# symek/facedeform

Hardware: AMD Instinct MI355X
Metric: deformed Mverts/sec at 256 ctrl pts, 1/2/4/8 MI355X vs host-CPU ref (higher is better)
Workload: dtype f32

## Files before the change

facedeform_amd/csrc/fd_capi.hip:

```cpp
#include <atomic>
#include <cstdarg>
#include <cstdio>
#include <cstdlib>
#include <cstring>
#include <initializer_list>
#include <new>

#include "fd_internal.h"

using namespace fd;

struct GraphKey {
    int M, kind, term, nparams;
    double params[4];
    const void *A, *rest, *rec32;
};

struct fd_batch;
struct fd_ctx {
    int device = 0;
    hipStream_t own_stream = nullptr;
    hipStream_t stream_ = nullptr;
    int eval_precision = FD_EVAL_FP32;
    int eval_variant = 0;
    int output = FD_OUTPUT_POSITION;
    int solver = FD_SOLVER_AUTO;
    int imported_layers = 0;
    uint64_t rig_build_id = 0;
    const float *rest_src = nullptr;
    bool prefer_lu = false;
    unsigned long long model_gen = 0;
    bool last_spd = false;
    bool last_nopivot = false;
    bool last_reg = false;

    int M = 0, kind = FD_KERNEL_GAUSSIAN_QNN, term = FD_TERM_LINEAR, nparams = 0;
    double params[4] = {1.0, 5.0, 0.0, 0.0};
    bool points_set = false;
    bool build_pending = false;
    bool built = false;
    bool have_report = false;
    fd_report report{};
    bool have_factor = false;
    bool factor_grouped = false;
    bool deltas_only = false;
    hipGraphExec_t resolve_exec = nullptr;

    int cap_M = 0;
    int cap_npad = 0;
    int cap_records = 0;
    float *d_rest = nullptr, *d_delta = nullptr;
    double *d_centres = nullptr, *d_radii = nullptr, *d_W = nullptr;
    double *d_A = nullptr, *d_X = nullptr;
    int *d_ipiv = nullptr, *d_moves = nullptr;
    Rec32 *d_rec32 = nullptr;
    Rec64 *d_rec64 = nullptr;
    MfmaTile *d_tiles = nullptr;
    MfmaTileH *d_tiles16 = nullptr;
    double *d_ns = nullptr;
    DevModel *d_model = nullptr;
    DevModel *h_model = nullptr;
    BatchSlot *d_slot = nullptr;
    BatchSlot h_slot{};
    uint64_t alloc_gen = 0;
    hipEvent_t wait_event = nullptr;
    hipStream_t wait_stream = nullptr;
    struct fd_batch *wait_batch = nullptr;
    hipEvent_t tev0 = nullptr, tev_mid = nullptr, tev1 = nullptr;
    ModelHeader *h_header = nullptr;
    int *h_status = nullptr;
    int *d_status_alias = nullptr;
    hipEvent_t status_ev = nullptr;
    hipEvent_t status_poll = nullptr;
    bool status_inflight = false;
    int sticky_rc = FD_OK;

    int64_t cap_N = 0;
    float *d_P = nullptr, *d_dist2 = nullptr, *d_fall = nullptr;
    float *d_tu = nullptr, *d_tv = nullptr, *d_nrm = nullptr;
    int64_t cap_vec = 0, cap_vecP = 0;
    float *d_vec = nullptr, *d_vecP = nullptr;
    int64_t mesh_N = 0, mesh_cap = 0;
    bool mesh_has_dist2 = false, mesh_has_frames = false;
    float *m_P = nullptr, *m_dist2 = nullptr, *m_tu = nullptr, *m_tv = nullptr, *m_nrm = nullptr;
    float *m_out = nullptr, *m_fall = nullptr;

    hipEvent_t ev0 = nullptr, ev_mid = nullptr, ev1 = nullptr;

    hipGraphExec_t build_exec = nullptr;
    bool use_graph = true;
    GraphKey graph_key{}, resolve_key{};
    char err[512] = {0};
};

struct ShotScratch {
    void *d = nullptr;
    size_t cap = 0;
    hipEvent_t consumed_ev = nullptr;
    bool consumed = false;
    hipEvent_t eval_ev = nullptr;
    bool eval_pending = false;
};

struct fd_batch {
    int n = 0;
    int device = 0;
    fd_ctx *ctxs[kMaxBatch] = {};
    uint64_t gens[kMaxBatch] = {};
    BatchSlot *d_slots = nullptr;
    PointSrc src{};
    bool have_src = false;
    hipEvent_t ev0 = nullptr, ev_mid = nullptr, ev1 = nullptr;
    hipGraphExec_t exec = nullptr;
    bool use_graph = true;
    GraphKey key{};
    hipStream_t waited_stream = nullptr;
    hipEvent_t status_ev = nullptr;
    struct SharedSet {
        void *d_wtiles = nullptr, *d_frames = nullptr;
        size_t cap_wtiles = 0, cap_frames = 0;
        hipEvent_t packed_ev = nullptr;
        hipEvent_t eval_ev = nullptr;
        hipEvent_t eval_done = nullptr;
        bool eval_pending = false;
    } sets[2];
    int *h_mismatch = nullptr;
    int eval_cus = 0;
    int shared_factor = 0;
    double *d_fac = nullptr;
    int last_shared_factor = 0;
    void *d_mlfac = nullptr;
    size_t cap_mlfac = 0;
    int cur_set = 0;
    bool packed_valid = false;
    bool prepared = false;
    unsigned long long prep_gen[kMaxBatch] = {0};
    float *prep_P_out[kMaxBatch] = {nullptr};
    float *prep_fall[kMaxBatch] = {nullptr};
    bool prep_has_fall = false;
    hipEvent_t fallback_ev = nullptr;
    ShotScratch s64;
    ShotScratch sml;
    ShotScratch sml64;
    hipEvent_t group_ev = nullptr;
    bool lean = false;
    hipEvent_t consumed_override = nullptr;
    char err[512] = {0};
};


static thread_local char g_err[512] = {0};

static void set_err(fd_ctx *ctx, const char *fmt, ...)
{
    char *dst = ctx ? ctx->err : g_err;
    va_list ap;
    va_start(ap, fmt);
    vsnprintf(dst, 512, fmt, ap);
    va_end(ap);
}

static hipStream_t cur_stream(fd_ctx *ctx)
{
    if (ctx->stream_) return ctx->stream_;
    if (!ctx->own_stream && hipStreamCreateWithFlags(&ctx->own_stream, hipStreamNonBlocking) != hipSuccess) {
        (void)hipGetLastError();
        ctx->own_stream = nullptr;
    }
    return ctx->own_stream;
}

#define FD_HIP(ctx, call)                                                               \
    do {                                                                                \
        hipError_t e_ = (call);                                                         \
        if (e_ != hipSuccess) {                                                         \
            set_err(ctx, "%s failed: %s (%s:%d)", #call, hipGetErrorString(e_), __FILE__, __LINE__); \
            return FD_E_DEVICE;                                                         \
        }                                                                               \
    } while (0)

static int use_device(fd_ctx *ctx)
{
    int cur = -1;
    FD_HIP(ctx, hipGetDevice(&cur));
    if (cur != ctx->device) FD_HIP(ctx, hipSetDevice(ctx->device));
    return FD_OK;
}

template <typename T>
static int dev_alloc(fd_ctx *ctx, T **p, size_t count)
{
    if (*p) { (void)hipFree(*p); *p = nullptr; }
    if (count == 0) count = 1;
    hipError_t e = hipMalloc((void **)p, count * sizeof(T));
    if (e != hipSuccess) {
        *p = nullptr;
        set_err(ctx, "hipMalloc(%zu bytes) failed: %s", count * sizeof(T), hipGetErrorString(e));
        return FD_E_NOMEM;
    }
    return FD_OK;
}

static int order_of(const fd_ctx *ctx) { return ctx->M + term_cols(ctx->term); }
static int ml_layers(const fd_ctx *ctx) { return ctx->kind == FD_KERNEL_GAUSSIAN_ML ? (int)ctx->params[1] : 0; }
static int model_centres(const fd_ctx *ctx) { return ctx->kind == FD_KERNEL_GAUSSIAN_ML ? ctx->M * ml_layers(ctx) : ctx->M; }
static int eval_kind(const fd_ctx *ctx) { return ctx->kind == FD_KERNEL_GAUSSIAN_ML ? FD_KERNEL_GAUSSIAN_QNN : ctx->kind; }
static int record_layers(const fd_ctx *ctx) { return ctx->kind == FD_KERNEL_GAUSSIAN_ML ? ml_layers(ctx) : ctx->imported_layers; }

static int ensure_records_capacity(fd_ctx *ctx, int n)
{
    int rc;
    if (n > ctx->cap_records) {
        const int npad = round_up(n, kRecPad);
        if ((rc = dev_alloc(ctx, &ctx->d_centres, (size_t)n * 3))) return rc;
        if ((rc = dev_alloc(ctx, &ctx->d_radii, (size_t)n))) return rc;
        if ((rc = dev_alloc(ctx, &ctx->d_W, (size_t)(n + 4) * 3))) return rc;
        if ((rc = dev_alloc(ctx, &ctx->d_rec32, (size_t)npad))) return rc;
        if ((rc = dev_alloc(ctx, &ctx->d_rec64, (size_t)npad))) return rc;
        if ((rc = dev_alloc(ctx, &ctx->d_tiles, (size_t)npad / 16))) return rc;
        if ((rc = dev_alloc(ctx, &ctx->d_tiles16, (size_t)npad / 16))) return rc;
        ctx->cap_records = n;
    }
    return FD_OK;
}

static int ensure_model_capacity(fd_ctx *ctx, int M)
{
// ... 1183 lines not shown
    if (!on_device) FD_HIP(ctx, hipStreamSynchronize(cur_stream(ctx)));
    ctx->have_factor = false;
    ctx->deltas_only = false;
    ++ctx->model_gen;
    ctx->points_set = false;
    ctx->rig_build_id = 0;
    ctx->rest_src = h.rig_token ? (const float *)(uintptr_t)(h.rig_token | 1u) : nullptr;
    ctx->build_pending = false;
    ctx->built = true;
    fd_report r{};
    r.terminationtype = 1;
    r.n = order_of(ctx);
    ctx->report = r;
    ctx->have_report = true;
    return FD_OK;
}

static void batch_err(fd_batch *b, const char *fmt, ...)
{
    char *dst = b ? b->err : g_err;
    va_list ap;
    va_start(ap, fmt);
    vsnprintf(dst, 512, fmt, ap);
    va_end(ap);
}

fd_batch *fd_batch_create(fd_ctx *const *ctxs, int n)
{
    if (!ctxs || n <= 0 || n > kMaxBatch) { set_err(nullptr, "fd_batch_create: need 1..%d contexts", kMaxBatch); return nullptr; }
    for (int i = 0; i < n; ++i) {
        if (!ctxs[i] || ctxs[i]->device != ctxs[0]->device) { set_err(nullptr, "fd_batch_create: contexts must exist and share one device"); return nullptr; }
        for (int j = 0; j < i; ++j)
            if (ctxs[j] == ctxs[i]) { set_err(nullptr, "fd_batch_create: context listed twice"); return nullptr; }
    }
    fd_batch *b = new (std::nothrow) fd_batch();
    if (!b) { set_err(nullptr, "fd_batch_create: out of host memory"); return nullptr; }
    b->n = n;
    b->device = ctxs[0]->device;
    for (int i = 0; i < n; ++i) b->ctxs[i] = ctxs[i];
    bool ok = hipSetDevice(b->device) == hipSuccess;
    ok = ok && hipMalloc((void **)&b->d_slots, sizeof(BatchSlot) * (size_t)n) == hipSuccess;
    ok = ok && hipEventCreate(&b->ev0) == hipSuccess && hipEventCreate(&b->ev_mid) == hipSuccess &&
         hipEventCreate(&b->ev1) == hipSuccess;
    ok = ok && hipEventCreateWithFlags(&b->status_ev, hipEventDisableTiming) == hipSuccess;
    ok = ok && hipHostMalloc((void **)&b->h_mismatch, sizeof(int), hipHostMallocMapped) == hipSuccess;
    if (ok) *b->h_mismatch = 0;
    if (!ok) {
        set_err(nullptr, "fd_batch_create: device resource allocation failed: %s", hipGetErrorString(hipGetLastError()));
        fd_batch_destroy(b);
        return nullptr;
    }
    return b;
}

static void shot_free(ShotScratch &sc)
{
    if (sc.d) (void)hipFree(sc.d);
    if (sc.consumed_ev) (void)hipEventDestroy(sc.consumed_ev);
    if (sc.eval_ev) (void)hipEventDestroy(sc.eval_ev);
}

void fd_batch_destroy(fd_batch *b)
{
    if (!b) return;
    (void)hipSetDevice(b->device);
    for (int i = 0; i < b->n; ++i) {
        fd_ctx *c = b->ctxs[i];
        if (c && c->wait_event == b->ev1) {
            if (c->wait_stream) (void)hipStreamSynchronize(c->wait_stream);
            c->wait_event = nullptr; c->wait_stream = nullptr; c->wait_batch = nullptr;
        }
        if (c && c->tev0 == b->ev0) { c->tev0 = c->ev0; c->tev_mid = c->ev_mid; c->tev1 = c->ev1; }
        if (c && (c->status_poll == b->status_ev || c->status_poll == b->ev1)) { c->status_poll = c->status_ev; c->status_inflight = false; }
    }
    if (b->status_ev) (void)hipEventDestroy(b->status_ev);
    if (b->exec) (void)hipGraphExecDestroy(b->exec);
    if (b->d_slots) (void)hipFree(b->d_slots);
    for (auto &st : b->sets) {
        if (st.d_wtiles) (void)hipFree(st.d_wtiles);
        if (st.d_frames) (void)hipFree(st.d_frames);
        if (st.packed_ev) (void)hipEventDestroy(st.packed_ev);
        if (st.eval_ev) (void)hipEventDestroy(st.eval_ev);
    }
    if (b->d_fac) (void)hipFree(b->d_fac);
    if (b->d_mlfac) (void)hipFree(b->d_mlfac);
    if (b->fallback_ev) (void)hipEventDestroy(b->fallback_ev);
    for (ShotScratch *sc : {&b->s64, &b->sml, &b->sml64}) shot_free(*sc);
    if (b->group_ev) (void)hipEventDestroy(b->group_ev);
    if (b->h_mismatch) (void)hipHostFree(b->h_mismatch);
    if (b->ev0) (void)hipEventDestroy(b->ev0);
    if (b->ev_mid) (void)hipEventDestroy(b->ev_mid);
    if (b->ev1) (void)hipEventDestroy(b->ev1);
    delete b;
}

const char *fd_batch_last_error(const fd_batch *b) { return b ? b->err : g_err; }

int fd_batch_set_points_dev(fd_batch *b, const float *const *d_rest_xyz, const float *const *d_delta_xyz, int M)
{
    if (!b || !d_rest_xyz || !d_delta_xyz) return FD_E_INVALID;
    if (M <= 0 || M + 4 > kMaxOrder) { batch_err(b, "fd_batch_set_points_dev: M = %d outside 1..%d", M, kMaxOrder - 4); return FD_E_INVALID; }
    b->prepared = false;
    if (b->h_mismatch && *b->h_mismatch != 0) {
        const int who = *b->h_mismatch - 1;
        *b->h_mismatch = 0;
        batch_err(b, "shared-rig evaluation of the previous group: context %d was built on other rest points than context 0 (same "
                     "address, other contents); its frame was passed through", who);
        return FD_E_INVALID;
    }
    for (int i = 0; i < b->n; ++i)
        if (!d_rest_xyz[i] || !d_delta_xyz[i]) { batch_err(b, "fd_batch_set_points_dev: null array for context %d", i); return FD_E_INVALID; }
    for (int i = 0; i < b->n; ++i) {
        fd_ctx *c = b->ctxs[i];
        int rc = use_device(c);
        if (!rc) rc = ensure_model_capacity(c, M);
        if (rc) { batch_err(b, "context %d: %s", i, c->err); return rc; }
        c->M = M;
        c->points_set = true;
        c->built = false;
        c->build_pending = false;
        c->have_factor = false;
        c->deltas_only = false;
        c->rest_src = d_rest_xyz[i];
        c->rig_build_id = 0;
        b->src.rest[i] = d_rest_xyz[i];
        b->src.delta[i] = d_delta_xyz[i];
    }
    b->have_src = true;
    return FD_OK;
}

int fd_batch_build_async(fd_batch *b, void *hip_stream)
{
    if (!b) return FD_E_INVALID;
    b->prepared = false;
    fd_ctx *c0 = b->ctxs[0];
    int rc = use_device(c0);
    if (rc) { batch_err(b, "%s", c0->err); return rc; }
    hipStream_t stream = hip_stream ? (hipStream_t)hip_stream : cur_stream(c0);
    for (int i = 0; i < b->n; ++i) {
        fd_ctx *c = b->ctxs[i];
        if (!c->points_set) { batch_err(b, "fd_batch_build: context %d has no control points", i); return FD_E_INVALID; }
        c->imported_layers = 0;
        if (!same_model(c, c0)) {
            batch_err(b, "fd_batch_build: context %d differs from context 0 in M, kernel, parameters or term", i);
            return FD_E_INVALID;
        }
    }
    const int npad = round_up(order_of(c0), 32);
    bool table_stale = false;
    for (int i = 0; i < b->n; ++i) {
        fd_ctx *c = b->ctxs[i];
        const bool grew = npad > c->cap_npad;
        if ((rc = ensure_solver_capacity(c, npad)) || (rc = ensure_records_capacity(c, model_centres(c))) || (rc = sync_slot(c))) {
            batch_err(b, "context %d: %s", i, c->err);
            return rc;
        }
        if (grew) {
            const size_t cols = (size_t)c->cap_npad + kRhsCols + 16;
            hipError_t e = hipMemsetAsync(c->d_A, 0, sizeof(double) * (size_t)c->cap_npad * cols, stream);
            if (e != hipSuccess) { batch_err(b, "hipMemsetAsync failed: %s", hipGetErrorString(e)); return FD_E_DEVICE; }
        }
        if (b->gens[i] != c->alloc_gen) table_stale = true;
    }
    if (table_stale) {
        BatchSlot tab[kMaxBatch];
// ... 9 lines not shown
    bb.reg_front = (b->eval_cus <= 0 || b->eval_cus >= (int)device_cus()) ? 1 : 0;
    bb.group_panels = b->n >= 4 ? 1 : 0;

    bool same_rest_launch = b->have_src;
    for (int i = 1; i < b->n && same_rest_launch; ++i) same_rest_launch = b->src.rest[i] == b->src.rest[0];
    bool shared_ml = b->shared_factor != 0 && bb.ml_layers > 0 && same_rest_launch && ml_shared_applies(bb.M, bb.ml_layers, b->n);
    if (shared_ml && ml_shared_init() != hipSuccess) { (void)hipGetLastError(); shared_ml = false; }
    if (shared_ml && ml_shared_scratch_bytes(bb) > b->cap_mlfac) {
        if (b->d_mlfac) (void)hipFree(b->d_mlfac);
        b->d_mlfac = nullptr; b->cap_mlfac = 0;
        if (hipMalloc(&b->d_mlfac, ml_shared_scratch_bytes(bb)) != hipSuccess) { (void)hipGetLastError(); b->d_mlfac = nullptr; shared_ml = false; }
        else b->cap_mlfac = ml_shared_scratch_bytes(bb);
    }

    const GraphKey key = graph_key(c0, (bb.spd << 9) | (bb.small << 10) | (bb.reg << 11) | (bb.nopivot << 12), false);
    if (!bb.reg && !shared_ml && b->use_graph &&
        ensure_graph(stream, &b->exec, &b->key, key, [&] { return launch_build(bb, stream, nullptr); }) != hipSuccess)
        b->use_graph = false;
#define FD_BHIP(call)                                                                         \
    do {                                                                                      \
        hipError_t e_ = (call);                                                               \
        if (e_ != hipSuccess) { batch_err(b, "%s failed: %s", #call, hipGetErrorString(e_)); return FD_E_DEVICE; } \
    } while (0)
    const bool shared_fac_ok = same_rest_launch;
    bool shared_fac = b->shared_factor != 0 && bb.reg && shared_fac_ok && b->n > 1;
    if (shared_fac && !b->d_fac && hipMalloc((void **)&b->d_fac, sizeof(double) * reg_factor_doubles()) != hipSuccess) {
        (void)hipGetLastError(); b->d_fac = nullptr; shared_fac = false;
    }
    b->last_shared_factor = (shared_fac || shared_ml) ? 1 : 0;
    if (!b->lean) FD_BHIP(hipEventRecord(b->ev0, stream));
    if (shared_fac) {
        FD_BHIP(launch_build_reg_shared(bb, stream, &b->src, nullptr, b->d_fac));
        b->have_src = false;
    } else if (bb.reg) {
        FD_BHIP(launch_build_reg(bb, stream, b->have_src ? &b->src : nullptr, nullptr));
        b->have_src = false;
    } else {
    FD_BHIP(launch_prepare(bb, stream, b->have_src ? &b->src : nullptr));
    b->have_src = false;
    if (shared_ml) {
        FD_BHIP(hipEventRecord(b->ev_mid, stream));
        FD_BHIP(launch_build_ml_shared(bb, stream, b->d_mlfac));
    } else if (b->use_graph && b->exec) {
        FD_BHIP(hipEventRecord(b->ev_mid, stream));
        FD_BHIP(hipGraphLaunch(b->exec, stream));
    } else {
        FD_BHIP(launch_build(bb, stream, b->ev_mid));
    }
    }
    if (!b->lean) FD_BHIP(hipEventRecord(b->ev1, stream));
    b->waited_stream = nullptr;
#undef FD_BHIP
    static std::atomic<uint64_t> build_ids{0};
    const uint64_t this_build = same_rest_launch ? ++build_ids : 0;
    hipEvent_t t0 = b->lean ? nullptr : b->ev0, t_mid = b->lean ? nullptr : (bb.reg ? b->ev0 : b->ev_mid), t1 = b->lean ? nullptr : b->ev1;
    for (int i = 0; i < b->n; ++i) note_build_enqueued(b->ctxs[i], b->ev1, stream, b, t0, t_mid, t1, &bb, this_build);
    arm_status(b->ctxs, b->n, stream, bb.reg != 0, b->ev1, b->status_ev);
    return FD_OK;
}

static int batch_poll(fd_batch *b)
{
    if (b->h_mismatch && *b->h_mismatch != 0) {
        batch_err(b, "shared-rig evaluation: context %d was built on other rest points than context 0 (same address, other "
                     "contents); its frame was passed through", *b->h_mismatch - 1);
        return FD_E_INVALID;
    }
    bool any = false;
    for (int i = 0; i < b->n; ++i) any = any || b->ctxs[i]->status_inflight || b->ctxs[i]->sticky_rc != FD_OK;
    if (!any) return FD_OK;
    bool shared_pending = false;
    hipEvent_t shared_ev = nullptr;
    for (int i = 0; i < b->n; ++i)
        if (b->ctxs[i]->status_inflight && (b->ctxs[i]->status_poll == b->status_ev || b->ctxs[i]->status_poll == b->ev1)) {
            shared_pending = true; shared_ev = b->ctxs[i]->status_poll;
        }
    if (shared_pending) {
        const hipError_t q = hipEventQuery(shared_ev);
        if (q == hipErrorNotReady) { (void)hipGetLastError(); return FD_OK; }
    }
    for (int i = 0; i < b->n; ++i) {
        const bool lu_before = b->ctxs[i]->prefer_lu;
        const int rc = poll_status(b->ctxs[i]);
        if (b->ctxs[i]->prefer_lu != lu_before) b->prepared = false;
        if (rc) { batch_err(b, "context %d: %s", i, b->ctxs[i]->err); return rc; }
    }
    return FD_OK;
}

int fd_batch_build_result(fd_batch *b, fd_report *reports)
{
    if (!b) return FD_E_INVALID;
    int first = FD_OK;
    for (int i = 0; i < b->n; ++i) {
        const int rc = fd_build_result(b->ctxs[i], reports ? &reports[i] : nullptr);
        if (rc && !first) { first = rc; batch_err(b, "context %d: %s", i, b->ctxs[i]->err); }
    }
    return first;
}

int fd_batch_deform_dev(fd_batch *b, void *hip_stream, int64_t N, const float *const *d_P_in, float *const *d_P_out,
                        const float *const *d_dist2, float *const *d_falloff_out, const float *const *d_tu,
                        const float *const *d_tv, const float *const *d_nrm, float radius2, float falloffrate)
{
    if (!b || !d_P_in || !d_P_out) return FD_E_INVALID;
    if (N < 0) { batch_err(b, "fd_batch_deform_dev: N < 0"); return FD_E_INVALID; }
    if (!frames_ok(d_tu, d_tv, d_nrm)) { batch_err(b, "fd_batch_deform_dev: tu, tv, nrm tables must be all set or all NULL"); return FD_E_INVALID; }
    if (N == 0) return FD_OK;
    fd_ctx *c0 = b->ctxs[0];
    int rc = use_device(c0);
    if (rc) { batch_err(b, "%s", c0->err); return rc; }
    hipStream_t stream = hip_stream ? (hipStream_t)hip_stream : cur_stream(c0);
    DeformArgs args[kMaxBatch];
    for (int i = 0; i < b->n; ++i) {
        fd_ctx *c = b->ctxs[i];
        if (!d_P_in[i] || !d_P_out[i]) { batch_err(b, "fd_batch_deform_dev: NULL vertex array for context %d", i); return FD_E_INVALID; }
        if (!c->built && !c->build_pending) { batch_err(b, "fd_batch_deform_dev: context %d has no built model", i); return FD_E_NOT_BUILT; }
        const float *tu = d_tu ? d_tu[i] : nullptr, *tv = d_tv ? d_tv[i] : nullptr, *nr = d_nrm ? d_nrm[i] : nullptr;
        if (!frames_ok(tu, tv, nr)) { batch_err(b, "fd_batch_deform_dev: context %d: tu, tv, nrm must be all set or all NULL", i); return FD_E_INVALID; }
        args[i] = deform_args(c, N, d_P_in[i], d_P_out[i], d_dist2 ? d_dist2[i] : nullptr, d_falloff_out ? d_falloff_out[i] : nullptr,
                              tu, tv, nr, radius2, falloffrate);
        if (c->output != c0->output) { batch_err(b, "fd_batch_deform_dev: context %d has another fd_set_output setting than context 0", i); return FD_E_INVALID; }
    }
    if ((rc = batch_poll(b))) return rc;
    for (int i = 0; i < b->n; ++i)
        if ((rc = order_after_batch(b->ctxs[i], stream))) { batch_err(b, "context %d: %s", i, b->ctxs[i]->err); return rc; }
    hipError_t e = launch_deform_batch(args, b->n, stream);
    if (e != hipSuccess) { batch_err(b, "launch_deform_batch failed: %s", hipGetErrorString(e)); return FD_E_DEVICE; }
    return FD_OK;
}

static int shared_applies(fd_batch *b, const char *who, float *const *d_P_out, int *ek_out)
{
    fd_ctx *c0 = b->ctxs[0];
    const int ek = eval_kind(c0);
    *ek_out = ek;
    bool fast = (ek == FD_KERNEL_THIN_PLATE || ek == FD_KERNEL_GAUSSIAN || ek == FD_KERNEL_GAUSSIAN_QNN) && round_up(c0->M, kRecPad) >= 32;
    for (int i = 0; i < b->n; ++i) {
        fd_ctx *c = b->ctxs[i];
        if (!d_P_out[i]) { batch_err(b, "%s: NULL output array for context %d", who, i); return FD_E_INVALID; }
        if (!c->built && !c->build_pending) { batch_err(b, "%s: context %d has no built model", who, i); return FD_E_NOT_BUILT; }
        if (!c->rest_src || c->rest_src != c0->rest_src || !same_model(c, c0)) {
            batch_err(b, "%s: the contexts must share one rest rig (fd_batch_set_points_dev with the "
                         "same rest array for all), kernel and term; context %d does not", who, i);
            return FD_E_INVALID;
        }
        if (c->output != c0->output) { batch_err(b, "%s: context %d has another fd_set_output setting than context 0", who, i); return FD_E_INVALID; }
        if (c->eval_precision != FD_EVAL_FP32 || c->eval_variant > 0 || record_layers(c) != 0) fast = false;
    }
    return fast ? 1 : 0;
}

static bool make_event(hipEvent_t *ev)
{
    if (*ev) return true;
    if (hipEventCreateWithFlags(ev, hipEventDisableTiming) != hipSuccess) { (void)hipGetLastError(); *ev = nullptr; return false; }
    return true;
}

static int shot_check_mesh(fd_batch *b, const char *who, int64_t N, const float *d_P_in, const float *d_tu, const float *d_tv,
                           const float *d_nrm)
{
    if (N < 0 || (N > 0 && !d_P_in)) { batch_err(b, "%s: bad N / P_in", who); return FD_E_INVALID; }
    if (!frames_ok(d_tu, d_tv, d_nrm)) { batch_err(b, "%s: tu, tv, nrm must be all set or all NULL", who); return FD_E_INVALID; }
    return FD_OK;
}

// ... 36 lines not shown
    for (int t = 0; t < 6; ++t) {
        if (!tabs[t]) continue;
        for (int i = 0; i < b->n; ++i) {
            const void *o = tabs[t][i];
            if (!o) { batch_err(b, "%s: output table %d has a NULL entry for context %d", who, t, i); return FD_E_INVALID; }
            for (const void *in : ins)
                if (in && o == in) { batch_err(b, "%s: an output of context %d is a shared input array", who, i); return FD_E_INVALID; }
        }
    }
    return FD_OK;
}

static int shot_begin(fd_batch *b, const char *who, ShotScratch &sc, hipStream_t stream)
{
    int rc;
    if (!b->lean && (rc = batch_poll(b))) return rc;
    for (int i = 0; i < b->n; ++i)
        if ((rc = order_after_batch(b->ctxs[i], stream))) { batch_err(b, "context %d: %s", i, b->ctxs[i]->err); return rc; }
    if (!make_event(&sc.consumed_ev)) { batch_err(b, "%s: hipEventCreate failed", who); return FD_E_DEVICE; }
    return FD_OK;
}

static int shot_reserve(fd_batch *b, const char *who, ShotScratch &sc, size_t bytes, hipStream_t stream)
{
    if (bytes > sc.cap) {
        if (sc.d) (void)hipFree(sc.d);
        sc.d = nullptr; sc.cap = 0; sc.eval_pending = false;
        if (hipMalloc(&sc.d, bytes) != hipSuccess) {
            (void)hipGetLastError();
            batch_err(b, "%s: scratch allocation (%zu bytes) failed", who, bytes);
            return FD_E_NOMEM;
        }
        sc.cap = bytes;
    }
    if (sc.eval_pending && hipStreamWaitEvent(stream, sc.eval_ev, 0) != hipSuccess) {
        batch_err(b, "%s: hipStreamWaitEvent failed: %s", who, hipGetErrorString(hipGetLastError()));
        return FD_E_DEVICE;
    }
    sc.eval_pending = false;
    return FD_OK;
}

static void shot_evaluated(ShotScratch &sc, hipStream_t stream)
{
    sc.consumed = true;
    if (make_event(&sc.eval_ev) && hipEventRecord(sc.eval_ev, stream) == hipSuccess) { sc.eval_pending = true; return; }
    (void)hipGetLastError();
    (void)hipStreamSynchronize(stream);
}

static void shot_vectors_evaluated(ShotScratch &sc, hipStream_t stream)
{
    if (sc.eval_pending && hipEventRecord(sc.eval_ev, stream) == hipSuccess) return;
    (void)hipGetLastError();
    (void)hipStreamSynchronize(stream);
}

static bool one_build(const fd_batch *b)
{
    const uint64_t id = b->ctxs[0]->rig_build_id;
    if (id == 0) return false;
    for (int i = 1; i < b->n; ++i)
        if (b->ctxs[i]->rig_build_id != id) return false;
    return true;
}

static int vectors_per_context(fd_batch *b, hipStream_t stream, int precision, hipEvent_t consumed_ev, int64_t N, const float *d_P_in,
                               float *const *d_P_out, const float *d_dist2, float *const *d_falloff_out, const float *d_tu,
                               const float *d_tv, const float *d_nrm, float radius2, float falloffrate, const fd_batch_vectors *vec)
{
    for (int i = 0; i < b->n; ++i) {
        DeformArgs a = deform_args(b->ctxs[i], N, d_P_in, d_P_out[i], d_dist2, d_falloff_out ? d_falloff_out[i] : nullptr, d_tu, d_tv,
                                   d_nrm, radius2, falloffrate);
        a.precision = precision;
        const VectorArgs v{vec->N, vec->tu, vec->tv, vec->N ? vec->N_out[i] : nullptr, vec->tu ? vec->tu_out[i] : nullptr,
                           vec->tv ? vec->tv_out[i] : nullptr, vec->jacobian ? vec->jacobian[i] : nullptr};
        hipError_t e = launch_vectors(a, v, stream);
        if (e != hipSuccess) { batch_err(b, "launch_vectors failed: %s", hipGetErrorString(e)); return FD_E_DEVICE; }
    }
    if (hipEventRecord(consumed_ev, stream) != hipSuccess) { (void)hipGetLastError(); return FD_E_DEVICE; }
    return FD_OK;
}

static int shared_pack(fd_batch *b, hipStream_t stream, int ek, float *const *d_P_out, float *const *d_falloff_out)
{
    fd_ctx *c0 = b->ctxs[0];
    const int si = b->packed_valid ? (b->cur_set ^ 1) : 0;
    fd_batch::SharedSet &st = b->sets[si];
    SharedDeformArgs a{};
    a.N = 1; a.Mpad = round_up(c0->M, kRecPad); a.nF = b->n; a.kind = ek; a.ctiles = c0->d_tiles16;
    a.falloff_out = d_falloff_out;
    int rc;
    if (!b->lean && (rc = batch_poll(b))) return rc;
    for (int i = 0; i < b->n; ++i) {
        fd_ctx *c = b->ctxs[i];
        a.rec32[i] = c->d_rec32; a.model[i] = c->d_model; a.P_out[i] = d_P_out[i]; a.centres[i] = c->d_centres;
        if ((rc = order_after_batch(c, stream))) { batch_err(b, "context %d: %s", i, c->err); return rc; }
    }
    {
        bool one_build = c0->rig_build_id != 0;
        for (int i = 1; i < b->n && one_build; ++i) one_build = b->ctxs[i]->rig_build_id == c0->rig_build_id;
        if (one_build) for (int i = 1; i < b->n; ++i) a.centres[i] = a.centres[0];
    }
    const size_t wb = shared_wtile_bytes(a.Mpad, a.nF), fb = shared_frame_bytes(a.nF);
    if (wb > st.cap_wtiles || fb > st.cap_frames) {
        if (st.d_wtiles) (void)hipFree(st.d_wtiles);
        if (st.d_frames) (void)hipFree(st.d_frames);
        st.d_wtiles = st.d_frames = nullptr; st.cap_wtiles = st.cap_frames = 0; st.eval_pending = false;
        if (hipMalloc(&st.d_wtiles, wb) != hipSuccess || hipMalloc(&st.d_frames, fb) != hipSuccess) {
            (void)hipGetLastError();
            batch_err(b, "shared-rig evaluation: scratch allocation (%zu bytes) failed", wb + fb);
            return FD_E_NOMEM;
        }
        st.cap_wtiles = wb; st.cap_frames = fb;
    }
    if (st.eval_pending && st.eval_done && hipStreamWaitEvent(stream, st.eval_done, 0) != hipSuccess) {
        batch_err(b, "shared-rig evaluation: hipStreamWaitEvent failed: %s", hipGetErrorString(hipGetLastError()));
        return FD_E_DEVICE;
    }
    st.eval_pending = false;
    a.wtiles = st.d_wtiles; a.frames = st.d_frames;
    a.packed_ev = b->lean ? nullptr : (make_event(&st.packed_ev) ? st.packed_ev : nullptr);
    b->consumed_override = nullptr;
    a.mode = 1;
    a.M = c0->M;
    if (b->h_mismatch && hipHostGetDevicePointer((void **)&a.mismatch, b->h_mismatch, 0) != hipSuccess) { (void)hipGetLastError(); a.mismatch = nullptr; }
    hipError_t e = launch_deform_shared(a, stream);
    if (e != hipSuccess) { batch_err(b, "launch_deform_shared (pack) failed: %s", hipGetErrorString(e)); return FD_E_DEVICE; }
    b->cur_set = si;
    b->packed_valid = b->lean || st.packed_ev != nullptr;
    b->prepared = true;
    for (int i = 0; i < b->n; ++i) {
        b->prep_P_out[i] = d_P_out[i]; b->prep_fall[i] = d_falloff_out ? d_falloff_out[i] : nullptr;
        b->prep_gen[i] = b->ctxs[i]->model_gen;
    }
    b->prep_has_fall = d_falloff_out != nullptr;
    return FD_OK;
}

int fd_batch_prepare_shared(fd_batch *b, void *hip_stream, float *const *d_P_out, float *const *d_falloff_out)
{
    if (!b || !d_P_out) return FD_E_INVALID;
    fd_ctx *c0 = b->ctxs[0];
    int rc = use_device(c0);
    if (rc) { batch_err(b, "%s", c0->err); return rc; }
    hipStream_t stream = hip_stream ? (hipStream_t)hip_stream : cur_stream(c0);
    int ek = 0;
    const int applies = shared_applies(b, "fd_batch_prepare_shared", d_P_out, &ek);
    if (applies < 0) return applies;
    if (applies == 0) return FD_OK;
    return shared_pack(b, stream, ek, d_P_out, d_falloff_out);
}

int fd_batch_deform_shared_dev(fd_batch *b, void *hip_stream, int64_t N, const float *d_P_in, float *const *d_P_out,
                               const float *d_dist2, float *const *d_falloff_out, const float *d_tu,
                               const float *d_tv, const float *d_nrm, float radius2, float falloffrate)
{
    if (!b || !d_P_out) return FD_E_INVALID;
    int rc = shot_check_mesh(b, "fd_batch_deform_shared_dev", N, d_P_in, d_tu, d_tv, d_nrm);
    if (rc) return rc;
    if (N == 0) return FD_OK;
    fd_ctx *c0 = b->ctxs[0];
    rc = use_device(c0);
    if (rc) { batch_err(b, "%s", c0->err); return rc; }
    hipStream_t stream = hip_stream ? (hipStream_t)hip_stream : cur_stream(c0);
    int ek = 0;
    const int applies = shared_applies(b, "fd_batch_deform_shared_dev", d_P_out, &ek);
    if (applies < 0) return applies;
    if (applies == 0) {
        const float *pin[kMaxBatch], *pd2[kMaxBatch], *ptu[kMaxBatch], *ptv[kMaxBatch], *pnr[kMaxBatch];
        for (int i = 0; i < b->n; ++i) { pin[i] = d_P_in; pd2[i] = d_dist2; ptu[i] = d_tu; ptv[i] = d_tv; pnr[i] = d_nrm; }
        rc = fd_batch_deform_dev(b, hip_stream, N, pin, d_P_out, d_dist2 ? pd2 : nullptr, d_falloff_out, d_tu ? ptu : nullptr,
                                 d_tu ? ptv : nullptr, d_tu ? pnr : nullptr, radius2, falloffrate);
        if (rc == FD_OK && make_event(&b->fallback_ev)) {
            if (hipEventRecord(b->fallback_ev, stream) != hipSuccess) { (void)hipGetLastError(); rc = FD_E_DEVICE; }
            b->packed_valid = false;
            b->consumed_override = nullptr;
        }
        return rc;
    }
    bool reuse = b->prepared && b->prep_has_fall == (d_falloff_out != nullptr);
    for (int i = 0; reuse && i < b->n; ++i)
        reuse = b->prep_P_out[i] == d_P_out[i] && (!d_falloff_out || b->prep_fall[i] == d_falloff_out[i]) &&
                b->prep_gen[i] == b->ctxs[i]->model_gen;
    if (reuse) {
        if (!b->lean && (rc = batch_poll(b))) return rc;
        if (!b->prepared) reuse = false;
        for (int i = 0; reuse && i < b->n; ++i)
            if ((rc = order_after_batch(b->ctxs[i], stream))) { batch_err(b, "context %d: %s", i, b->ctxs[i]->err); return rc; }
    }
    if (reuse) {
        fd_batch::SharedSet &ps = b->sets[b->cur_set];
        if (!b->lean && ps.packed_ev && hipStreamWaitEvent(stream, ps.packed_ev, 0) != hipSuccess) {
            batch_err(b, "fd_batch_deform_shared_dev: hipStreamWaitEvent failed: %s", hipGetErrorString(hipGetLastError()));
            return FD_E_DEVICE;
        }
    } else if ((rc = shared_pack(b, stream, ek, d_P_out, d_falloff_out))) {
        return rc;
    }
    fd_batch::SharedSet &st = b->sets[b->cur_set];
    SharedDeformArgs a{};
    a.N = N; a.P_in = d_P_in; a.dist2 = d_dist2; a.tu = d_tu; a.tv = d_tv; a.nrm = d_nrm;
    a.radius2 = radius2; a.falloffrate = falloffrate;
    a.Mpad = round_up(c0->M, kRecPad); a.nF = b->n;
    a.ctiles = c0->d_tiles16;
    a.kind = ek;
    a.falloff_out = d_falloff_out;
    for (int i = 0; i < b->n; ++i) { a.rec32[i] = b->ctxs[i]->d_rec32; a.model[i] = b->ctxs[i]->d_model; a.P_out[i] = d_P_out[i]; }
    a.wtiles = st.d_wtiles; a.frames = st.d_frames;
    a.packed_ev = nullptr;
    a.mode = 2;
    a.delta_out = c0->output == FD_OUTPUT_DISPLACEMENT;
    a.max_wgs = b->eval_cus;
    hipError_t e = launch_deform_shared(a, stream);
    if (e != hipSuccess) { batch_err(b, "launch_deform_shared failed: %s", hipGetErrorString(e)); return FD_E_DEVICE; }
    if (b->lean) {
        st.eval_done = b->ev1;
        st.eval_pending = true;
    } else if (make_event(&st.eval_ev)) {
        st.eval_done = st.eval_ev;
        if (hipEventRecord(st.eval_ev, stream) != hipSuccess) { (void)hipGetLastError(); st.eval_pending = false; }
        else st.eval_pending = true;
    } else {
        (void)hipStreamSynchronize(stream);
    }
    return FD_OK;
}

int fd_batch_deform_vectors_shared_dev(fd_batch *b, void *hip_stream, int64_t N, const float *d_P_in, float *const *d_P_out,
                                       const float *d_dist2, float *const *d_falloff_out, const float *d_tu, const float *d_tv,
                                       const float *d_nrm, float radius2, float falloffrate, const fd_batch_vectors *vec)
{
    if (!b || !d_P_out) return FD_E_INVALID;
    const char *who = "fd_batch_deform_vectors_shared_dev";
    bool want;
    int rc = shot_check_vectors(b, who, N, d_P_in, d_P_out, d_dist2, d_falloff_out, d_tu, d_tv, d_nrm, vec, &want);
    if (rc) return rc;
    if (!want)
        return fd_batch_deform_shared_dev(b, hip_stream, N, d_P_in, d_P_out, d_dist2, d_falloff_out, d_tu, d_tv, d_nrm, radius2, falloffrate);
    if (N == 0) return FD_OK;
    fd_ctx *c0 = b->ctxs[0];
    rc = use_device(c0);
    if (rc) { batch_err(b, "%s", c0->err); return rc; }
    hipStream_t stream = hip_stream ? (hipStream_t)hip_stream : cur_stream(c0);
    int ek = 0;
    const int applies = shared_applies(b, who, d_P_out, &ek);
    if (applies < 0) return applies;
    if (applies == 0) {
        for (int i = 0; i < b->n; ++i) {
            fd_ctx *c = b->ctxs[i];
            const fd_vectors v{(int)sizeof(fd_vectors), vec->N, vec->N ? vec->N_out[i] : nullptr, vec->tu, vec->tu ? vec->tu_out[i] : nullptr,
                               vec->tv, vec->tv ? vec->tv_out[i] : nullptr, vec->jacobian ? vec->jacobian[i] : nullptr};
            rc = deform_dev_common(c, stream, N, d_P_in, d_P_out[i], d_dist2, d_falloff_out ? d_falloff_out[i] : nullptr, d_tu, d_tv, d_nrm,
                                   radius2, falloffrate, &v);
            if (rc) { batch_err(b, "context %d: %s", i, c->err); return rc; }
        }
        if (make_event(&b->fallback_ev)) {
            if (hipEventRecord(b->fallback_ev, stream) != hipSuccess) { (void)hipGetLastError(); return FD_E_DEVICE; }
            b->packed_valid = false;
            b->consumed_override = nullptr;
        }
        return FD_OK;
    }
    if ((rc = fd_batch_deform_shared_dev(b, hip_stream, N, d_P_in, d_P_out, d_dist2, d_falloff_out, d_tu, d_tv, d_nrm, radius2, falloffrate)))
        return rc;
    fd_batch::SharedSet &st = b->sets[b->cur_set];
    SharedVectorArgs a{};
    fill_mesh(a, N, d_P_in, d_dist2, d_tu, d_tv, d_nrm, radius2, falloffrate);
    a.Mpad = round_up(c0->M, kRecPad); a.nF = b->n; a.kind = ek;
    fill_vector_tables(a, b->n, vec);
    a.wtiles = st.d_wtiles; a.frames = st.d_frames;
    a.max_wgs = b->eval_cus;
    hipError_t e = launch_vectors_shared(a, stream);
    if (e != hipSuccess) { batch_err(b, "launch_vectors_shared failed: %s", hipGetErrorString(e)); return FD_E_DEVICE; }
    if (st.eval_pending && st.eval_done == st.eval_ev && st.eval_ev && hipEventRecord(st.eval_ev, stream) != hipSuccess) {
        (void)hipGetLastError();
        (void)hipStreamSynchronize(stream);
    }
    return FD_OK;
}

const char *fd_shared_vectors_kernel_name(int M, int frames, int kind)
{
    const char *pos = fd_shared_kernel_name(M, frames, kind);
    return pos[0] ? shared_vectors_kernel_name(round_up(M, kRecPad), frames, kind) : "";
}

static bool shared64_kind(int kind)
{
    return kind == FD_KERNEL_THIN_PLATE || kind == FD_KERNEL_GAUSSIAN || kind == FD_KERNEL_GAUSSIAN_QNN || kind == FD_KERNEL_BIHARMONIC ||
           kind == FD_KERNEL_CUBIC;
}

static bool shared64_fast(const fd_batch *b)
{
    const fd_ctx *c0 = b->ctxs[0];
    bool fast = shared64_kind(eval_kind(c0)) && c0->kind != FD_KERNEL_GAUSSIAN_ML;
    for (int i = 0; i < b->n; ++i)
        if (b->ctxs[i]->eval_variant > 0 || record_layers(b->ctxs[i]) != 0) fast = false;
    return fast;
}

int fd_batch_deform_shared_fp64_dev(fd_batch *b, void *hip_stream, int64_t N, const float *d_P_in, float *const *d_P_out,
                                    const float *d_dist2, float *const *d_falloff_out, const float *d_tu, const float *d_tv,
                                    const float *d_nrm, float radius2, float falloffrate)
{
    if (!b || !d_P_out) return FD_E_INVALID;
    const char *who = "fd_batch_deform_shared_fp64_dev";
    int rc = shot_check_mesh(b, who, N, d_P_in, d_tu, d_tv, d_nrm);
    if (!rc) rc = shot_check_aliasing(b, who, d_P_in, d_P_out, d_dist2, d_falloff_out, d_tu, d_tv, d_nrm);
    if (rc) return rc;
    if (N == 0) return FD_OK;
    fd_ctx *c0 = b->ctxs[0];
    rc = use_device(c0);
    if (rc) { batch_err(b, "%s", c0->err); return rc; }
    hipStream_t stream = hip_stream ? (hipStream_t)hip_stream : cur_stream(c0);
    const bool fast = shared64_fast(b);
    for (int i = 0; i < b->n; ++i) {
        fd_ctx *c = b->ctxs[i];
        if (!c->built && !c->build_pending) { batch_err(b, "%s: context %d has no built model", who, i); return FD_E_NOT_BUILT; }
        if (!c->rest_src || c->rest_src != c0->rest_src || !same_model(c, c0)) {
            batch_err(b, "%s: the contexts must share one rest rig (fd_batch_set_points_dev with the "
                         "same rest array for all), kernel and term; context %d does not", who, i);
            return FD_E_INVALID;
        }
        if (c->output != c0->output) { batch_err(b, "%s: context %d has another fd_set_output setting than context 0", who, i); return FD_E_INVALID; }
    }
    ShotScratch &sc = b->s64;
    if ((rc = shot_begin(b, who, sc, stream))) return rc;
    if (!fast) {
        for (int i = 0; i < b->n; ++i) {
            DeformArgs a = deform_args(b->ctxs[i], N, d_P_in, d_P_out[i], d_dist2, d_falloff_out ? d_falloff_out[i] : nullptr, d_tu, d_tv,
                                       d_nrm, radius2, falloffrate);
            a.precision = FD_EVAL_FP64;
            hipError_t e = launch_deform(a, stream);
            if (e != hipSuccess) { batch_err(b, "launch_deform failed: %s", hipGetErrorString(e)); return FD_E_DEVICE; }
        }
        if (hipEventRecord(sc.consumed_ev, stream) != hipSuccess) { (void)hipGetLastError(); return FD_E_DEVICE; }
        sc.consumed = true;
        return FD_OK;
    }
    Shared64Args a{};
    fill_mesh(a, N, d_P_in, d_dist2, d_tu, d_tv, d_nrm, radius2, falloffrate);
    a.M = c0->M; a.Mpad = round_up(c0->M, kRecPad); a.nF = b->n; a.kind = eval_kind(c0);
    const bool same_rig = one_build(b);
    for (int i = 0; i < b->n; ++i) {
        fd_ctx *c = b->ctxs[i];
        a.rec64[i] = c->d_rec64; a.model[i] = c->d_model; a.P_out[i] = d_P_out[i];
        a.centres[i] = same_rig ? c0->d_centres : c->d_centres;
    }
    a.falloff_out = d_falloff_out;
    a.delta_out = c0->output == FD_OUTPUT_DISPLACEMENT;
    a.max_wgs = b->eval_cus;
    const size_t bytes = shared64_scratch_bytes(a.Mpad, a.nF);
    if ((rc = shot_reserve(b, who, sc, bytes, stream))) return rc;
    a.scratch = sc.d;
    a.packed_ev = sc.consumed_ev;
    if (b->h_mismatch && hipHostGetDevicePointer((void **)&a.mismatch, b->h_mismatch, 0) != hipSuccess) { (void)hipGetLastError(); a.mismatch = nullptr; }
    hipError_t e = launch_deform_shared64(a, stream);
    if (e != hipSuccess) { batch_err(b, "launch_deform_shared64 failed: %s", hipGetErrorString(e)); return FD_E_DEVICE; }
// ... 223 lines not shown
    a.M = c0->M; a.layers = ml_layers(c0); a.nF = b->n;
    fill_vector_tables(a, b->n, vec);
    a.scratch = b->sml64.d;
    a.max_wgs = b->eval_cus;
    hipError_t e = launch_vectors_shared_ml64(a, stream);
    if (e != hipSuccess) { batch_err(b, "launch_vectors_shared_ml64 failed: %s", hipGetErrorString(e)); return FD_E_DEVICE; }
    shot_vectors_evaluated(b->sml64, stream);
    return FD_OK;
}

const char *fd_shared_vectors_ml_fp64_kernel_name(int M, int layers, int frames)
{
    return shared_vectors_ml64_kernel_name(M, layers, frames);
}

int fd_batch_wait_consumed(fd_batch *b, void *hip_stream)
{
    if (!b) return FD_E_INVALID;
    hipEvent_t ev = b->consumed_override ? b->consumed_override : (b->packed_valid ? b->sets[b->cur_set].packed_ev : b->fallback_ev);
    hipEvent_t evs[4] = {ev, nullptr, nullptr, nullptr};
    int n_ev = ev ? 1 : 0;
    for (const ShotScratch *sc : {&b->s64, &b->sml, &b->sml64})
        if (sc->consumed) evs[n_ev++] = sc->consumed_ev;
    if (n_ev == 0) return FD_OK;
    fd_ctx *c0 = b->ctxs[0];
    int rc = use_device(c0);
    if (rc) { batch_err(b, "%s", c0->err); return rc; }
    hipStream_t stream = hip_stream ? (hipStream_t)hip_stream : cur_stream(c0);
    for (int i = 0; i < n_ev; ++i)
        if (hipStreamWaitEvent(stream, evs[i], 0) != hipSuccess) {
            batch_err(b, "fd_batch_wait_consumed: hipStreamWaitEvent failed: %s", hipGetErrorString(hipGetLastError()));
            return FD_E_DEVICE;
        }
    return FD_OK;
}

int fd_batch_cook_group(fd_batch *b, void *build_stream, void *eval_stream, const float *d_rest_xyz,
                        const float *const *d_delta_xyz, int M, int64_t N, const float *d_P_in, float *const *d_P_out,
                        float *const *d_falloff_out, const fd_group_events *events)
{
    if (!b || !d_rest_xyz || !d_delta_xyz || !d_P_out) return FD_E_INVALID;
    fd_ctx *c0 = b->ctxs[0];
    hipStream_t bs = build_stream ? (hipStream_t)build_stream : cur_stream(c0);
    hipStream_t es = eval_stream ? (hipStream_t)eval_stream : bs;
    auto mark = [&](void *ev, hipStream_t st) { if (ev && hipEventRecord((hipEvent_t)ev, st) != hipSuccess) (void)hipGetLastError(); };
#ifdef FD_TUNING
    static const bool cook_timing = tuning_env("FD_COOK_TIMING") != nullptr;
    struct CookClock {
        bool on; double t[6]; int n = 0;
        static double now() { timespec ts; clock_gettime(CLOCK_MONOTONIC, &ts); return ts.tv_sec * 1e6 + ts.tv_nsec * 1e-3; }
        void tick() { if (on && n < 6) t[n++] = now(); }
        ~CookClock() { if (on && n == 6) fprintf(stderr, "[cook_group host us] wait_consumed %.1f | set_points %.1f | build %.1f | packing %.1f | evaluation %.1f\n", t[1] - t[0], t[2] - t[1], t[3] - t[2], t[4] - t[3], t[5] - t[4]); }
    } clk{cook_timing};
#define FD_COOK_TICK() clk.tick()
#else
#define FD_COOK_TICK()
#endif
    FD_COOK_TICK();
    int rc = fd_batch_wait_consumed(b, build_stream);
    if (rc) return rc;
    FD_COOK_TICK();
    const float *rest[kMaxBatch];
    for (int i = 0; i < b->n; ++i) rest[i] = d_rest_xyz;
    if ((rc = fd_batch_set_points_dev(b, rest, d_delta_xyz, M))) return rc;
    const bool lean = es == bs;
    struct LeanScope {
        fd_batch *b; hipStream_t s; bool on, built = false;
        ~LeanScope() {
            if (!on) return;
            if (built && hipEventRecord(b->ev1, s) != hipSuccess) (void)hipGetLastError();
            b->prepared = false;
            b->lean = false;
        }
    } scope{b, bs, lean};
    b->lean = lean;
    FD_COOK_TICK();
    if (events) mark(events->before_build, bs);
    if ((rc = fd_batch_build_async(b, build_stream))) return rc;
    scope.built = true;
    if (events) mark(events->after_build, bs);
    FD_COOK_TICK();
    if ((rc = fd_batch_prepare_shared(b, build_stream, d_P_out, d_falloff_out))) return rc;
    FD_COOK_TICK();
    if (es != bs) {
        if (!make_event(&b->group_ev) || hipEventRecord(b->group_ev, bs) != hipSuccess || hipStreamWaitEvent(es, b->group_ev, 0) != hipSuccess) {
            batch_err(b, "fd_batch_cook_group: ordering the evaluation stream failed: %s", hipGetErrorString(hipGetLastError()));
            return FD_E_DEVICE;
        }
    }
    if (events) mark(events->before_eval, es);
    rc = fd_batch_deform_shared_dev(b, es, N, d_P_in, d_P_out, nullptr, d_falloff_out, nullptr, nullptr, nullptr, 1.0f, 1.0f);
    if (events) mark(events->after_eval, es);
    FD_COOK_TICK();
    if (lean && rc == FD_OK && b->packed_valid && b->sets[b->cur_set].eval_pending) b->consumed_override = b->ev1;
    return rc;
}

int fd_batch_set_eval_cus(fd_batch *b, int n_cus)
{
    if (!b) return FD_E_INVALID;
    b->eval_cus = n_cus > 0 ? n_cus : 0;
    return FD_OK;
}

int fd_batch_set_shared_factor(fd_batch *b, int on)
{
    if (!b) return FD_E_INVALID;
    b->shared_factor = on ? 1 : 0;
    return FD_OK;
}

int fd_batch_last_build_shared_factor(const fd_batch *b) { return b ? b->last_shared_factor : 0; }

const char *fd_shared_ml_build_kernel_name(int M, int layers, int frames) { return ml_shared_kernel_name(M, layers, frames); }

int fd_batch_size(const fd_batch *b) { return b ? b->n : 0; }

const char *fd_shared_kernel_name(int M, int frames, int kind)
{
    const bool takes = (kind == FD_KERNEL_THIN_PLATE || kind == FD_KERNEL_GAUSSIAN || kind == FD_KERNEL_GAUSSIAN_QNN) && M > 0 && round_up(M, kRecPad) >= 32 &&
                       frames >= 1 && frames <= kMaxBatch;
    return takes ? shared_kernel_name(round_up(M, kRecPad), frames, kind) : "";
}

}
```

Measured before the change: 63740.

## Widen shared-set ring to eight and batch eval-done events with a guard

Grows the shared packed-weight ring from two to eight sets. It replaces the per-launch eval event record with one shared guard event, recorded only every few launches or when a set is about to be reused. In cook_group, when the pack was already done on the build stream, the eval stream waits only on the pack event instead of a full group event, which skips redundant per-context ordering. The goal is to cut per-call event-record and cross-stream wait overhead in the host-bound shared-rig path, at the cost of more device memory and more complex bookkeeping around reuse hazards.

```diff
diff --git a/facedeform_amd/csrc/fd_capi.hip b/facedeform_amd/csrc/fd_capi.hip
--- a/facedeform_amd/csrc/fd_capi.hip
+++ b/facedeform_amd/csrc/fd_capi.hip
@@ -1,4 +1,5 @@
 #include <atomic>
+#include <cassert>
 #include <cstdarg>
 #include <cstdio>
 #include <cstdlib>
@@ -102,6 +103,8 @@
     bool eval_pending = false;
 };
 
+static constexpr int kSharedSets = 8;
+
 struct fd_batch {
     int n = 0;
     int device = 0;
@@ -122,8 +125,14 @@
         hipEvent_t packed_ev = nullptr;
         hipEvent_t eval_ev = nullptr;
         hipEvent_t eval_done = nullptr;
+        uint64_t read_no = 0;
         bool eval_pending = false;
-    } sets[2];
+    } sets[kSharedSets];
+    hipStream_t eval_stream = nullptr;
+    uint64_t launch_no = 0;
+    hipEvent_t guard_ev = nullptr;
+    uint64_t guard_no = 0;
+    bool own_event_next = false;
     int *h_mismatch = nullptr;
     int eval_cus = 0;
     int shared_factor = 0;
@@ -143,6 +152,7 @@
     ShotScratch sml;
     ShotScratch sml64;
     hipEvent_t group_ev = nullptr;
+    bool pack_behind_build = false;
     bool lean = false;
     hipEvent_t consumed_override = nullptr;
     char err[512] = {0};
@@ -1492,6 +1502,7 @@
         if (st.packed_ev) (void)hipEventDestroy(st.packed_ev);
         if (st.eval_ev) (void)hipEventDestroy(st.eval_ev);
     }
+    if (b->guard_ev) (void)hipEventDestroy(b->guard_ev);
     if (b->d_fac) (void)hipFree(b->d_fac);
     if (b->d_mlfac) (void)hipFree(b->d_mlfac);
     if (b->fallback_ev) (void)hipEventDestroy(b->fallback_ev);
@@ -1667,7 +1678,7 @@
     for (int i = 0; i < b->n; ++i) {
         const bool lu_before = b->ctxs[i]->prefer_lu;
         const int rc = poll_status(b->ctxs[i]);
-        if (b->ctxs[i]->prefer_lu != lu_before) b->prepared = false;
+        if (b->ctxs[i]->prefer_lu != lu_before) { b->prepared = false; b->own_event_next = true; }
         if (rc) { batch_err(b, "context %d: %s", i, b->ctxs[i]->err); return rc; }
     }
     return FD_OK;
@@ -1870,10 +1881,24 @@
     return FD_OK;
 }
 
+static void sets_take_own_events(fd_batch *b)
+{
+    if (!b->guard_ev) return;
+    bool failed = false;
+    for (auto &st : b->sets) {
+        if (!st.eval_pending || st.eval_done != b->guard_ev) continue;
+        if (make_event(&st.eval_ev) && hipEventRecord(st.eval_ev, b->eval_stream) == hipSuccess) { st.eval_done = st.eval_ev; continue; }
+        (void)hipGetLastError();
+        st.eval_pending = false;
+        failed = true;
+    }
+    if (failed) (void)hipDeviceSynchronize();
+}
+
 static int shared_pack(fd_batch *b, hipStream_t stream, int ek, float *const *d_P_out, float *const *d_falloff_out)
 {
     fd_ctx *c0 = b->ctxs[0];
-    const int si = b->packed_valid ? (b->cur_set ^ 1) : 0;
+    const int si = b->packed_valid ? (b->cur_set + 1) % kSharedSets : 0;
     fd_batch::SharedSet &st = b->sets[si];
     SharedDeformArgs a{};
     a.N = 1; a.Mpad = round_up(c0->M, kRecPad); a.nF = b->n; a.kind = ek; a.ctiles = c0->d_tiles16;
@@ -1901,8 +1926,19 @@
             return FD_E_NOMEM;
         }
         st.cap_wtiles = wb; st.cap_frames = fb;
-    }
-    if (st.eval_pending && st.eval_done && hipStreamWaitEvent(stream, st.eval_done, 0) != hipSuccess) {
+        b->own_event_next = true;
+    }
+    hipEvent_t done = st.eval_pending ? st.eval_done : nullptr;
+    if (done && done == b->guard_ev) {
+#ifdef FD_TUNING
+        assert(b->launch_no - st.read_no < (uint64_t)(kSharedSets - 1) || b->guard_no >= st.read_no);
+#endif
+        if (b->guard_no < st.read_no) {
+            if (hipEventRecord(b->guard_ev, b->eval_stream) == hipSuccess) b->guard_no = b->launch_no;
+            else { (void)hipGetLastError(); (void)hipDeviceSynchronize(); done = nullptr; }
+        }
+    }
+    if (done && hipStreamWaitEvent(stream, done, 0) != hipSuccess) {
         batch_err(b, "shared-rig evaluation: hipStreamWaitEvent failed: %s", hipGetErrorString(hipGetLastError()));
         return FD_E_DEVICE;
     }
@@ -1974,19 +2010,22 @@
     if (reuse) {
         if (!b->lean && (rc = batch_poll(b))) return rc;
         if (!b->prepared) reuse = false;
-        for (int i = 0; reuse && i < b->n; ++i)
+        for (int i = 0; reuse && !b->pack_behind_build && i < b->n; ++i)
             if ((rc = order_after_batch(b->ctxs[i], stream))) { batch_err(b, "context %d: %s", i, b->ctxs[i]->err); return rc; }
     }
     if (reuse) {
         fd_batch::SharedSet &ps = b->sets[b->cur_set];
-        if (!b->lean && ps.packed_ev && hipStreamWaitEvent(stream, ps.packed_ev, 0) != hipSuccess) {
+        if (!b->lean && !b->pack_behind_build && ps.packed_ev && hipStreamWaitEvent(stream, ps.packed_ev, 0) != hipSuccess) {
             batch_err(b, "fd_batch_deform_shared_dev: hipStreamWaitEvent failed: %s", hipGetErrorString(hipGetLastError()));
             return FD_E_DEVICE;
         }
+        if (b->pack_behind_build) b->waited_stream = stream;
     } else if ((rc = shared_pack(b, stream, ek, d_P_out, d_falloff_out))) {
         return rc;
     }
     fd_batch::SharedSet &st = b->sets[b->cur_set];
+    const bool moved = b->launch_no > 0 && b->eval_stream != stream;
+    if (moved || b->lean) sets_take_own_events(b);
     SharedDeformArgs a{};
     a.N = N; a.P_in = d_P_in; a.dist2 = d_dist2; a.tu = d_tu; a.tv = d_tv; a.nrm = d_nrm;
     a.radius2 = radius2; a.falloffrate = falloffrate;
@@ -2002,9 +2041,21 @@
     a.max_wgs = b->eval_cus;
     hipError_t e = launch_deform_shared(a, stream);
     if (e != hipSuccess) { batch_err(b, "launch_deform_shared failed: %s", hipGetErrorString(e)); return FD_E_DEVICE; }
+    const uint64_t no = ++b->launch_no;
+    st.read_no = no;
+    b->eval_stream = stream;
+    const bool own_event = moved || b->own_event_next;
+    if (!b->lean) b->own_event_next = false;
     if (b->lean) {
         st.eval_done = b->ev1;
         st.eval_pending = true;
+    } else if (!own_event && make_event(&b->guard_ev)) {
+        st.eval_done = b->guard_ev;
+        st.eval_pending = true;
+        if (no - b->guard_no >= (uint64_t)(kSharedSets / 2)) {
+            if (hipEventRecord(b->guard_ev, stream) == hipSuccess) b->guard_no = no;
+            else (void)hipGetLastError();
+        }
     } else if (make_event(&st.eval_ev)) {
         st.eval_done = st.eval_ev;
         if (hipEventRecord(st.eval_ev, stream) != hipSuccess) { (void)hipGetLastError(); st.eval_pending = false; }
@@ -2061,9 +2112,14 @@
     a.max_wgs = b->eval_cus;
     hipError_t e = launch_vectors_shared(a, stream);
     if (e != hipSuccess) { batch_err(b, "launch_vectors_shared failed: %s", hipGetErrorString(e)); return FD_E_DEVICE; }
-    if (st.eval_pending && st.eval_done == st.eval_ev && st.eval_ev && hipEventRecord(st.eval_ev, stream) != hipSuccess) {
-        (void)hipGetLastError();
-        (void)hipStreamSynchronize(stream);
+    if (st.eval_pending && st.eval_done && st.eval_done != b->ev1) {
+        if (make_event(&st.eval_ev) && hipEventRecord(st.eval_ev, stream) == hipSuccess) {
+            st.eval_done = st.eval_ev;
+        } else {
+            (void)hipGetLastError();
+            (void)hipStreamSynchronize(stream);
+            st.eval_pending = false;
+        }
     }
     return FD_OK;
 }
@@ -2453,14 +2509,22 @@
     FD_COOK_TICK();
     if ((rc = fd_batch_prepare_shared(b, build_stream, d_P_out, d_falloff_out))) return rc;
     FD_COOK_TICK();
-    if (es != bs) {
+    const bool packed_here = es != bs && b->prepared && b->packed_valid && b->sets[b->cur_set].packed_ev != nullptr;
+    if (packed_here) {
+        if (hipStreamWaitEvent(es, b->sets[b->cur_set].packed_ev, 0) != hipSuccess) {
+            batch_err(b, "fd_batch_cook_group: ordering the evaluation stream failed: %s", hipGetErrorString(hipGetLastError()));
+            return FD_E_DEVICE;
+        }
+    } else if (es != bs) {
         if (!make_event(&b->group_ev) || hipEventRecord(b->group_ev, bs) != hipSuccess || hipStreamWaitEvent(es, b->group_ev, 0) != hipSuccess) {
             batch_err(b, "fd_batch_cook_group: ordering the evaluation stream failed: %s", hipGetErrorString(hipGetLastError()));
             return FD_E_DEVICE;
         }
     }
     if (events) mark(events->before_eval, es);
+    b->pack_behind_build = packed_here;
     rc = fd_batch_deform_shared_dev(b, es, N, d_P_in, d_P_out, nullptr, d_falloff_out, nullptr, nullptr, nullptr, 1.0f, 1.0f);
+    b->pack_behind_build = false;
     if (events) mark(events->after_eval, es);
     FD_COOK_TICK();
     if (lean && rc == FD_OK && b->packed_valid && b->sets[b->cur_set].eval_pending) b->consumed_override = b->ev1;
```

Result: no change. 64130, median of 3 (+0.6%).
